# philipjesic/Distributed-Proof-Of-Work

Hardware: AMD Instinct MI355X
Metric: MD5 candidates/sec (GH/s), whole node (higher is better)
Workload: dtype u32; 1 GPU; sweep: nonce [1,2,3,4], 32 trailing zeros (unreachable), 2^36 candidates per GPU per step in the L=4 chunk segment (k >= 2^24); per-step RCCL MIN all-reduce; ntz=32, parallelism=prefix-partition x1 (workerBits=0)

## Files before the change

### distributed-proof-of-work_amd/csrc/md5_launch_ctl.h

```cpp
#pragma once
#include "md5_kernel_tune.h"

namespace dpow {
namespace DPOW_KNS {

constexpr uint32_t kTraceWaves = 8192;
constexpr uint32_t kTraceFields = 8;
#if DPOW_WAVE_TRACE
static __device__ unsigned long long g_wave_trace[kTraceWaves * kTraceFields];
#define DPOW_TRACED(...) { __VA_ARGS__ }
#else
#define DPOW_TRACED(...) {}
#endif
struct WaveTrace {
    unsigned long long t_start, t_first, n_wb, t_last, c_last, reason, t_hit, t_claims, t_bar;
    static DPOW_DEV unsigned long long now() { return __builtin_amdgcn_s_memrealtime(); }
    DPOW_DEV void start() DPOW_TRACED(t_start = now(); t_first = n_wb = t_last = c_last = reason = t_hit = 0;)
    DPOW_DEV void first_claim(uint64_t claim) DPOW_TRACED(t_first = now() + (claim & 0);)
    DPOW_DEV void chunk(uint64_t claim) DPOW_TRACED(t_last = now(); c_last = claim;)
    DPOW_DEV void wave_block() DPOW_TRACED(++n_wb;)
    DPOW_DEV void hit(bool h) DPOW_TRACED(if (h && t_hit == 0) t_hit = now();)
    DPOW_DEV void left(uint32_t why) DPOW_TRACED(reason = why;)
    DPOW_DEV void store(uint32_t lane) DPOW_TRACED(
        const uint32_t wave = (blockIdx.x - 1u) * (kBlockThreads / 64) + threadIdx.x / 64u;
        if (lane == 0 && wave < kTraceWaves) {
            unsigned long long *w = g_wave_trace + kTraceFields * wave;
            w[0] = t_start; w[1] = t_first; w[2] = now(); w[3] = n_wb;
            w[4] = t_last; w[5] = c_last; w[6] = reason; w[7] = t_hit;
        })
    DPOW_DEV void claims_performed() DPOW_TRACED(t_claims = now();)
    DPOW_DEV void barrier_passed() DPOW_TRACED(t_bar = now();)
    DPOW_DEV void counted(const Launch &L, uint32_t prev, uint32_t n) DPOW_TRACED(
        if (prev + n == L.done_target) {
            unsigned long long *r = g_wave_trace + kTraceFields * (kTraceWaves - 2);
            r[0] = t_claims; r[1] = t_bar; r[2] = now() + (prev & 0);
        })
    static DPOW_DEV void released() DPOW_TRACED(g_wave_trace[kTraceFields * (kTraceWaves - 2) + 3] = now();)
    static DPOW_DEV void watch(int f) DPOW_TRACED(
        unsigned long long *w = g_wave_trace + kTraceFields * (kTraceWaves - 1);
        if (f == 0 || f == 3 || w[f] == 0) w[f] = now();
        if (f == 0) w[1] = w[2] = 0;)
};
#undef DPOW_TRACED

__device__ __attribute__((noinline)) void publish(Ctrl *ctrl, Snap *snap, uint32_t seq, unsigned long long *claim,
                                                  Ctrl *ctrl_next) {
    if (ctrl_next == nullptr) {
        constexpr uintptr_t kRingBytes = kCtrlRing * kCtrlStride * sizeof(Ctrl);
        const uintptr_t a = reinterpret_cast<uintptr_t>(ctrl);
        ctrl_next =
            reinterpret_cast<Ctrl *>((a & ~(kRingBytes - 1)) | ((a + kCtrlStride * sizeof(Ctrl)) & (kRingBytes - 1)));
    }
    const unsigned long long t_start = __hip_atomic_load(&claim[1], __ATOMIC_RELAXED, __HIP_MEMORY_SCOPE_AGENT);
    for (uint32_t x = 0; x < kClaimCounters; ++x) claim[x * kClaimStride] = 0ull;
    claim[1] = 0ull;
    ctrl_next->best = kNoHit;
    ctrl_next->stop = 0u;
    ctrl_next->done = 0u;
    const unsigned long long best = __hip_atomic_load(&ctrl->best, __ATOMIC_RELAXED, __HIP_MEMORY_SCOPE_AGENT);
    const uint32_t stop = __hip_atomic_load(&ctrl->stop, __ATOMIC_RELAXED, __HIP_MEMORY_SCOPE_AGENT);
    __hip_atomic_store(&snap->best, best, __ATOMIC_RELAXED, __HIP_MEMORY_SCOPE_SYSTEM);
    __hip_atomic_store(&snap->stop, stop, __ATOMIC_RELAXED, __HIP_MEMORY_SCOPE_SYSTEM);
    __hip_atomic_store(&snap->t_start, t_start, __ATOMIC_RELAXED, __HIP_MEMORY_SCOPE_SYSTEM);
    __hip_atomic_store(&snap->t_end, __builtin_amdgcn_s_memrealtime(), __ATOMIC_RELAXED, __HIP_MEMORY_SCOPE_SYSTEM);
    __hip_atomic_store(&snap->seq, seq, __ATOMIC_RELEASE, __HIP_MEMORY_SCOPE_SYSTEM);
    WaveTrace::released();
}

DPOW_DEV void retire(const Launch &L, uint32_t done, Ctrl *ctrl_next) {
    if (done == L.done_target) publish(L.ctrl, L.snap, L.seq, L.claim, ctrl_next);
}

DPOW_DEV void watcher(const Launch &L) {
    if (threadIdx.x != 0) return;
    __hip_atomic_store(&L.claim[1], __builtin_amdgcn_s_memrealtime(), __ATOMIC_RELAXED, __HIP_MEMORY_SCOPE_AGENT);
    unsigned long long node_seen = ~0ull, bound_seen = L.bound0, early_seen = kNoHit;
    WaveTrace::watch(0);
    for (;;) {
        const unsigned long long *const nbp = L.node_best ? L.node_best : L.ext_bound;
        const uint32_t *const nsp = L.node_stop ? L.node_stop : L.cancel;
        const uint32_t done = __hip_atomic_load(&L.ctrl->done, __ATOMIC_RELAXED, __HIP_MEMORY_SCOPE_AGENT);
        const unsigned long long b = __hip_atomic_load(&L.ctrl->best, __ATOMIC_RELAXED, __HIP_MEMORY_SCOPE_AGENT);
        const uint32_t stale = __hip_atomic_load(L.stale, __ATOMIC_RELAXED, __HIP_MEMORY_SCOPE_SYSTEM);
        const uint32_t cancel = __hip_atomic_load(L.cancel, __ATOMIC_RELAXED, __HIP_MEMORY_SCOPE_SYSTEM);
        const unsigned long long eb = __hip_atomic_load(L.ext_bound, __ATOMIC_RELAXED, __HIP_MEMORY_SCOPE_SYSTEM);
        const unsigned long long nb = __hip_atomic_load(nbp, __ATOMIC_RELAXED, __HIP_MEMORY_SCOPE_SYSTEM);
        const uint32_t nstop = __hip_atomic_load(nsp, __ATOMIC_RELAXED, __HIP_MEMORY_SCOPE_SYSTEM);
        if (done >= L.done_target) {
            WaveTrace::watch(3);
            return;
        }
        if (L.early && b < early_seen) {
            WaveTrace::watch(2);
            early_seen = b;
            __hip_atomic_store(L.early, b, __ATOMIC_RELAXED, __HIP_MEMORY_SCOPE_SYSTEM);
        }
        bool stop = cancel != 0u || (int32_t)(stale - L.seq) >= 0;
        if (eb < bound_seen) {
            bound_seen = eb;
            __hip_atomic_fetch_min(&L.ctrl->best, eb, __ATOMIC_RELAXED, __HIP_MEMORY_SCOPE_AGENT);
        }
        if (L.node_best) {
            if (nb < node_seen) {
                if (nb < kNoHit) WaveTrace::watch(1);
                node_seen = nb;
                __hip_atomic_fetch_min(&L.ctrl->best, nb, __ATOMIC_RELAXED, __HIP_MEMORY_SCOPE_AGENT);
            }
            stop = stop || nstop != 0u;
        }
        if (stop) {
            __hip_atomic_store(&L.ctrl->stop, 1u, __ATOMIC_RELAXED, __HIP_MEMORY_SCOPE_AGENT);
            return;
        }
        __builtin_amdgcn_s_sleep(kWatchSleep);
    }
}

template <bool kOpaque>
DPOW_DEV unsigned long long claim_issue(unsigned long long *ctr, uint32_t lane) {
    unsigned long long v = 0;
    if constexpr (kOpaque) {
        uint32_t z;
        asm volatile("v_mov_b32 %0, 0" : "=v"(z));
        ctr += z;
    }
    if (lane == 0) v = __hip_atomic_fetch_add(ctr, 1ull, __ATOMIC_RELAXED, __HIP_MEMORY_SCOPE_AGENT);
    return v;
}

DPOW_DEV uint64_t claim_take(unsigned long long v, uint32_t x, uint64_t base) {
    const uint32_t lo = __builtin_amdgcn_readfirstlane((uint32_t)v);
    const uint32_t hi = __builtin_amdgcn_readfirstlane((uint32_t)(v >> 32));
    return (((uint64_t)hi << 32) | lo) * kClaimCounters + x + base;
}

DPOW_DEV uint64_t claim_next(unsigned long long *ctr, uint32_t x, uint32_t lane, uint64_t base) {
    return claim_take(claim_issue<false>(ctr, lane), x, base);
}

DPOW_DEV uint64_t lane_range_mask(int64_t lo, int64_t hi) {
    lo = lo < 0 ? 0 : (lo > 64 ? 64 : lo);
    hi = hi < 0 ? 0 : (hi > 64 ? 64 : hi);
    if (hi <= lo) return 0;
    const uint64_t upto_hi = hi == 64 ? ~0ull : ((1ull << hi) - 1ull);
    const uint64_t below_lo = lo == 64 ? ~0ull : ((1ull << lo) - 1ull);
    return upto_hi & ~below_lo;
}

}
}
```

### distributed-proof-of-work_amd/csrc/md5_search_si.h

```cpp
#pragma once

namespace dpow {
namespace DPOW_KNS {

constexpr uint32_t kSegLimitNone = 0xFFFFFFFFu;

DPOW_DEV uint64_t local_ceil_of_global(uint64_t g, uint32_t rbits, uint32_t base_tb) {
    const uint64_t k = g >> 8;
    const uint32_t tb = (uint32_t)(g & 0xFFu);
    if (tb < base_tb) return k << rbits;
    const uint32_t t = tb - base_tb;
    return t >> rbits ? (k + 1u) << rbits : (k << rbits) + t;
}

struct SegLimit {
    uint32_t q, r;
};
DPOW_DEV SegLimit seg_limit_of(const Launch &L, unsigned long long best) {
    const uint32_t segbits = 24u + L.rbits;
    const uint64_t ib = local_ceil_of_global(best, L.rbits, L.base_tb);
    const uint64_t rel = ib > L.wb_begin ? ib - L.wb_begin : 0ull;
    const uint64_t q = rel >> segbits;
    SegLimit l;
    l.q = q >= (uint64_t)kSegLimitNone ? kSegLimitNone - 1u : (uint32_t)q;
    l.r = (uint32_t)(rel - (q << segbits));
    return l;
}
DPOW_DEV uint32_t seg_limit_at(const SegLimit &l, uint32_t o) { return l.q + (o < l.r ? 1u : 0u); }

template <int NBLK, int W0, int SH>
DPOW_DEV void seg_invariants(uint32_t (&x)[4][kNC], uint32_t (&p)[kNC], const Launch &L, VarWords<true> &v) {
#pragma unroll
    for (int j = 0; j < kNC; ++j) {
        x[0][j] = L.iv[0]; x[1][j] = L.iv[1]; x[2][j] = L.iv[2]; x[3][j] = L.iv[3];
    }
    md5_steps<NBLK, W0, SH, 0, 0, W0 + 1, kNC>(x, L, v);
    using R = Roles<W0 + 1>;
#pragma unroll
    for (int j = 0; j < kNC; ++j) {
        p[j] = x[R::a][j] + md5_fn<W0 + 1>(x[R::b][j], x[R::c][j], x[R::d][j]);
        asm volatile("" : "+v"(p[j]), "+v"(x[Roles<W0>::a][j]));
        asm volatile("" : "+v"(v.w0km[1][j]), "+v"(v.w0km[2][j]), "+v"(v.w0km[3][j]));
    }
}

template <int NBLK, int W0, int SH>
DPOW_DEV uint64_t hash_wave_block_si(const Launch &L, const KConst &kc, const uint32_t (&xin)[4][kNC],
                                     const uint32_t (&p)[kNC], const VarWords<true> &v, const uint32_t (&vs)[kNC],
                                     uint32_t s, uint32_t o, uint32_t lane, uint32_t loff) {
    using K = VgprK<NBLK, W0, SH, true>;
    static_assert(K::Tune::kLead >= 2, "steps W0 and W0 + 1 precede the hand-ordered pipeline");
    uint32_t x[4][kNC];
#pragma unroll
    for (int j = 0; j < kNC; ++j)
#pragma unroll
        for (int w = 0; w < 4; ++w) x[w][j] = xin[w][j];
    {
        using R = Roles<W0 + 1>;
        const uint32_t km = L.KT[W0 + 1] + v.seg_d[0];
#pragma unroll
        for (int j = 0; j < kNC; ++j) x[R::a][j] = x[R::b][j] + __builtin_rotateleft32(p[j] + km, md5_shift(W0 + 1));
    }
    md5_steps<NBLK, W0, SH, 0, W0 + 2, K::kI0, kNC>(x, L, v);
    pipe::steps<NBLK, W0, SH, 0, K::kI0, K::kEnd0>(x, L, v);

    uint64_t bal[kNC];
    uint64_t any = 0;
#pragma unroll
    for (int j = 0; j < kNC; ++j) {
        bal[j] = __ballot(x[3][j] == L.deq);
        any |= bal[j];
    }
    if (any != 0) {
        const uint64_t i0 = L.wb_begin + ((uint64_t)s << (24u + L.rbits)) + o;
#pragma unroll
        for (int j = 0; j < kNC; ++j) {
            const uint64_t ij = i0 + 64u * j;
            uint64_t m = bal[j] & lane_range_mask((int64_t)(L.i_begin - ij), (int64_t)(L.i_end - ij));
            if (m != 0 && L.ntz > 8u) {
                const uint32_t sd[3] = {v.seg_d[0], 0u, 0u};
                const bool ok = ((m >> lane) & 1ull) && full_check<NBLK, W0, SH, true>(L, kc, vs[j], loff, sd);
                m = __ballot(ok);
            }
            if (m != 0) {
                const uint64_t g = global_of_local(ij + (uint64_t)__builtin_ctzll(m), L.rbits, L.base_tb);
                if (lane == 0) {
                    const unsigned long long prev = __hip_atomic_fetch_min(
                        &L.ctrl->best, (unsigned long long)g, __ATOMIC_RELAXED, __HIP_MEMORY_SCOPE_AGENT);
                    asm volatile("; dpow: atomicMin performed (%0)" ::"v"(prev));
                }
                return g;
            }
        }
    }
    return kNoHitG;
}

template <int NBLK, int W0, int SH, bool EQ>
DPOW_DEV void search_body_si(const Launch &L) {
    static_assert(NBLK == 1 && SH == 0 && EQ && W0 + 1 != 16 * NBLK - 2,
                  "segment-inner: one final block, SH = 0, D-equality, W0 + 1 not the bit-length word");
    if (blockIdx.x == 0) {
        watcher(L);
        return;
    }
    if constexpr (DPOW_SI_PAD > 0) asm volatile(".rept %0\n s_nop 0\n .endr" ::"i"(DPOW_SI_PAD));
    const uint32_t lane = threadIdx.x & 63u;
    const uint32_t loff = lane_offset(L.rbits, lane);
    KConst kc;
    kconst_init<NBLK, W0, SH, 0, 0, true>(kc, L);

    unsigned long long best = __hip_atomic_load(&L.ctrl->best, __ATOMIC_RELAXED, __HIP_MEMORY_SCOPE_AGENT);
    best = best < L.bound0 ? best : L.bound0;
    uint32_t stop = __hip_atomic_load(&L.ctrl->stop, __ATOMIC_RELAXED, __HIP_MEMORY_SCOPE_AGENT);

    __builtin_amdgcn_s_setprio(1);
    uint32_t x = (blockIdx.x - 1u) % kClaimCounters;
    const bool skip = stop != 0u || global_of_local(L.i_begin, L.rbits, L.base_tb) >= best;
    uint64_t claim = skip ? L.n_chunks : claim_next(L.claim + x * kClaimStride, x, lane, 0);
    const uint32_t segbits = 24u + L.rbits;
    SegLimit lim = seg_limit_of(L, best);
    uint32_t pc = L.poll_wb;
    unsigned long long best_seen = __hip_atomic_load(&L.ctrl->best, __ATOMIC_RELAXED, __HIP_MEMORY_SCOPE_AGENT);
    uint32_t stop_seen = __hip_atomic_load(&L.ctrl->stop, __ATOMIC_RELAXED, __HIP_MEMORY_SCOPE_AGENT);
    uint32_t hops = 0;
    for (;;) {
        if (claim >= L.n_chunks) {
            if (skip || ++hops >= kClaimCounters) break;
            x = (x + 1u) % kClaimCounters;
            const unsigned long long seen =
                __hip_atomic_load(L.claim + x * kClaimStride, __ATOMIC_RELAXED, __HIP_MEMORY_SCOPE_AGENT);
            claim = seen * kClaimCounters + x < L.n_chunks ? claim_next(L.claim + x * kClaimStride, x, lane, 0)
                                                           : L.n_chunks;
            continue;
        }
        unsigned long long next_v = 0;
        bool issued = false;
        const bool big = claim < L.n_big;
        if (!big) __builtin_amdgcn_s_setprio(0);
        const uint64_t b_begin = big ? claim * L.chunk : L.n_big * L.chunk + (claim - L.n_big) * L.chunk_tail;
        const uint32_t csz = big ? L.chunk : L.chunk_tail;
        const uint32_t nb = (uint32_t)(b_begin + csz < L.n_wblocks ? csz : L.n_wblocks - b_begin);
        uint32_t o = (uint32_t)(b_begin * (uint64_t)kWaveBlock);
        bool over = false;
        for (uint32_t left = nb; left != 0 && stop == 0u; --left, o += (uint32_t)kWaveBlock) {
            uint32_t s = L.wb_begin + o + (uint64_t)kWaveBlock <= L.i_begin ? 1u : 0u;
            const uint32_t s_hi =
                L.n_seg - (L.wb_begin + ((uint64_t)(L.n_seg - 1u) << segbits) + o >= L.i_end ? 1u : 0u);
            uint32_t s_end = seg_limit_at(lim, o);
            if (s_end == 0u) {
                over = true;
                break;
            }
            s_end = s_end < s_hi ? s_end : s_hi;
            if (left == 1u) {
                next_v = claim_issue<true>(L.claim + x * kClaimStride, lane);
                issued = true;
            }
            if (s >= s_end) continue;
            uint32_t vs[kNC];
            VarWords<true> v;
            v.kc = &kc;
            v.seg_d[0] = v.seg_d[1] = v.seg_d[2] = 0u;
#pragma unroll
            for (int j = 0; j < kNC; ++j) {
                vs[j] = wave_uniform_v(L.wb_begin + o + 64u * j, L.rbits, L.base_tb);
                var_words<SH>(v, j, vs[j], loff, 0u);
                w0km_fill<W0>(v, j, L);
            }
            uint32_t xin[4][kNC], p[kNC];
            seg_invariants<NBLK, W0, SH>(xin, p, L, v);
            for (; s < s_end; ++s) {
                v.seg_d[0] = s;
                if constexpr (DPOW_SI_VSEG != 0) {
                    const uint32_t d[3] = {s, 0u, 0u};
                    kconst_seg<NBLK, W0, SH, 0, 0, true>(kc, L, d);
                }
                const uint64_t g = hash_wave_block_si<NBLK, W0, SH>(L, kc, xin, p, v, vs, s, o, lane, loff);
                if (g != kNoHitG) {
                    best = g < best ? g : best;
                    lim = seg_limit_of(L, best);
                    s_end = s;
                }
                if (--pc == 0u) {
                    pc = L.poll_wb;
                    const bool lower = best_seen < best;
                    best = lower ? best_seen : best;
                    stop = stop_seen;
                    best_seen = __hip_atomic_load(&L.ctrl->best, __ATOMIC_RELAXED, __HIP_MEMORY_SCOPE_AGENT);
                    stop_seen = __hip_atomic_load(&L.ctrl->stop, __ATOMIC_RELAXED, __HIP_MEMORY_SCOPE_AGENT);
                    if (lower) {
                        lim = seg_limit_of(L, best);
                        const uint32_t e = seg_limit_at(lim, o);
                        s_end = e < s_end ? e : s_end;
                    }
                    if (stop != 0u) s_end = s;
                }
            }
        }
        if (stop != 0u || over || !issued) break;
        claim = claim_take(next_v, x, 0);
    }
    asm volatile("s_waitcnt vmcnt(0)" ::: "memory");
    __builtin_amdgcn_fence(__ATOMIC_RELEASE, "workgroup");
    __syncthreads();
    if (threadIdx.x == 0)
        retire(L, __hip_atomic_fetch_add(&L.ctrl->done, 1u, __ATOMIC_RELAXED, __HIP_MEMORY_SCOPE_AGENT) + 1u, L.ctrl_next);
}

}
}
```

### distributed-proof-of-work_amd/csrc/md5_variant.hip

```cpp
#include "md5_search_kernel.h"
#include "md5_variants.h"

#include <hip/hip_ext.h>

#ifndef DPOW_VNBLK
#error "DPOW_VNBLK must be defined"
#endif
#ifndef DPOW_VSH
#error "DPOW_VSH must be defined"
#endif

namespace dpow {

namespace {
using namespace DPOW_KNS;
using KernelFn = void (*)(Launch);
template <int NBLK, int W0, int SH, bool EQ, bool KSPAN>
constexpr KernelFn kernel_of() {
    constexpr int kSgpr = KernelTune<NBLK, W0, SH, KSPAN>::kSgpr;
    if constexpr (kSgpr == 2) return md5_search_kernel_w15sgpr<NBLK, W0, SH, EQ, KSPAN>;
    else if constexpr (kSgpr == 1) return md5_search_kernel_lsgpr<NBLK, W0, SH, EQ, KSPAN>;
    else return md5_search_kernel<NBLK, W0, SH, EQ, KSPAN>;
}
#define DPOW_K(w, e, nar) \
    kernel_of<DPOW_VNBLK, w, DPOW_VSH, e, !(DPOW_VSH == 3 && nar && narrow_knobs(DPOW_VNBLK, w).on)>()
#if DPOW_VSI
#if DPOW_VNBLK != 1 || DPOW_VSH != 0
#error "the segment-inner unit is built for NBLK = 1, SH = 0"
#endif
constexpr int kW0Lo = 0;
const KernelFn kTable[1][1][4] = {
    {{DPOW_K(0, true, false), DPOW_K(1, true, false), DPOW_K(2, true, false), DPOW_K(3, true, false)}}};
#define DPOW_ROW(e, n)
#elif DPOW_VNBLK == 1
constexpr int kW0Lo = 0;
#define DPOW_ROW(e, n)                                                                                              \
    {DPOW_K(0, e, n), DPOW_K(1, e, n), DPOW_K(2, e, n),  DPOW_K(3, e, n),  DPOW_K(4, e, n),  DPOW_K(5, e, n),        \
     DPOW_K(6, e, n), DPOW_K(7, e, n), DPOW_K(8, e, n),  DPOW_K(9, e, n),  DPOW_K(10, e, n), DPOW_K(11, e, n),       \
     DPOW_K(12, e, n), DPOW_K(13, e, n)}
const KernelFn kTable[2][2][14] = {{DPOW_ROW(false, false), DPOW_ROW(false, true)},
                                   {DPOW_ROW(true, false), DPOW_ROW(true, true)}};
#else
constexpr int kW0Lo = 12;
#define DPOW_ROW(e, n) {DPOW_K(12, e, n), DPOW_K(13, e, n), DPOW_K(14, e, n), DPOW_K(15, e, n)}
const KernelFn kTable[2][2][4] = {{DPOW_ROW(false, false), DPOW_ROW(false, true)},
                                  {DPOW_ROW(false, false), DPOW_ROW(false, true)}};
#endif
#undef DPOW_ROW
#undef DPOW_K
constexpr int kW0N = sizeof(kTable[0][0]) / sizeof(kTable[0][0][0]);

KernelFn pick(int w0, bool eq, bool narrow) {
#if DPOW_VSI
    return eq && w0 >= kW0Lo && w0 < kW0Lo + kW0N ? kTable[0][0][w0 - kW0Lo] : nullptr;
#endif
    return (w0 >= kW0Lo && w0 < kW0Lo + kW0N) ? kTable[eq ? 1 : 0][narrow ? 1 : 0][w0 - kW0Lo] : nullptr;
}
}

#if DPOW_VLS
#define DPOW_SFX _ls
#elif DPOW_VSI
#define DPOW_SFX _si
#else
#define DPOW_SFX
#endif
#define DPOW_CAT4(a, b, c, d) a##b##_##c##d
#define DPOW_NAME2(a, b, c, d) DPOW_CAT4(a, b, c, d)
#define DPOW_NAME(a, b, c) DPOW_NAME2(a, b, c, DPOW_SFX)

hipError_t DPOW_NAME(variant_launch_, DPOW_VNBLK, DPOW_VSH)(int w0, const Launch &L, uint32_t grid,
                                                           hipStream_t stream) {
    KernelFn fn = pick(w0, use_d_equality(DPOW_VNBLK, L.ntz), L.rbits >= 6u);
    if (!fn) return hipErrorInvalidValue;
    hipLaunchKernelGGL(fn, dim3(grid), dim3(kBlockThreads), 0, stream, L);
    return hipGetLastError();
}

hipError_t DPOW_NAME(variant_prepare_, DPOW_VNBLK, DPOW_VSH)() {
    for (const auto &eq : kTable)
        for (const auto &row : eq)
            for (KernelFn fn : row) {
                hipFuncAttributes a;
                const hipError_t e = hipFuncGetAttributes(&a, reinterpret_cast<const void *>(fn));
                if (e != hipSuccess) return e;
            }
    return hipSuccess;
}

hipError_t DPOW_NAME(variant_occupancy_, DPOW_VNBLK, DPOW_VSH)(int w0, int *blocks_per_cu) {
    KernelFn fn = pick(w0, DPOW_VSI != 0, true);
    if (!fn) return hipErrorInvalidValue;
    return hipOccupancyMaxActiveBlocksPerMultiprocessor(blocks_per_cu, reinterpret_cast<const void *>(fn),
                                                        kBlockThreads, 0);
}

}

#if DPOW_WAVE_TRACE && DPOW_VNBLK == 1 && DPOW_VSH == 0
#if DPOW_VLS
extern "C" int dpow_diag_wave_trace_ls(unsigned long long *out, size_t n) {
#else
extern "C" int dpow_diag_wave_trace(unsigned long long *out, size_t n) {
#endif
    if (n > dpow::DPOW_KNS::kTraceWaves * dpow::DPOW_KNS::kTraceFields)
        n = dpow::DPOW_KNS::kTraceWaves * dpow::DPOW_KNS::kTraceFields;
    return hipMemcpyFromSymbol(out, HIP_SYMBOL(dpow::DPOW_KNS::g_wave_trace), n * 8, 0, hipMemcpyDeviceToHost) == hipSuccess
               ? 0
               : -2;
}
#endif
```

### distributed-proof-of-work_amd/csrc/search.cpp

```cpp
#include <string.h>
#include <time.h>

#include <algorithm>

#include "ctx.h"
#include "md5_variants.h"

namespace dpow {

std::atomic<int> g_active[kMaxDevices];
std::mutex g_ctx_mu;
std::vector<dpow_ctx *> g_ctxs;

namespace {

constexpr int DPOW_BOUNDED = 3;

constexpr int64_t kSpinNs = 200000;
constexpr int64_t kSpinMaxNs = 4000000;
constexpr long kPollNs = 5000;
constexpr int64_t kNoDeadline = INT64_MAX;
constexpr int64_t kQueueLeadNs = 60000;
constexpr int64_t kEstFixedNs = 8000;

struct ActiveSearch {
    int dev;
    explicit ActiveSearch(int d) : dev(d) { g_active[dev].fetch_add(1, std::memory_order_relaxed); }
    ~ActiveSearch() { g_active[dev].fetch_sub(1, std::memory_order_relaxed); }
};

struct SearchWait {
    int64_t t0 = now_ns();
    int64_t spin_ns = kSpinNs;
    TimerSlack slack;
    uint64_t node_seen = DPOW_NO_HIT;
    bool node_stop = false;
    const uint64_t *early = nullptr;
    uint64_t early_seen = DPOW_NO_HIT;
    uint64_t own_posted = DPOW_NO_HIT;
    uint64_t covered = 0;
    const uint8_t *nonce = nullptr;
    size_t nonce_len = 0;
    uint32_t ntz = 0;
    uint32_t rbits = 8, base_tb = 0;
};

int poll_node(dpow_ctx *c, SearchWait &sw) {
    dpow_node_slot *n = c->node;
    if (!n) return 0;
    const uint64_t nb = __atomic_load_n(&n->best, __ATOMIC_ACQUIRE);
    if (nb < sw.node_seen) {
        sw.node_seen = nb;
        if (nb != sw.own_posted) {
            std::lock_guard<std::mutex> g(c->bound_mu);
            uint64_t cur = c->ext_bound.load(std::memory_order_relaxed);
            if (nb < cur) c->ext_bound.store(nb, std::memory_order_release);
        }
    }
    if (!sw.node_stop && __atomic_load_n(&n->stop, __ATOMIC_ACQUIRE) != 0u) {
        sw.node_stop = true;
        __atomic_store_n(&c->h_cancel[kStaleWord], (uint32_t)c->seq, __ATOMIC_RELEASE);
    }
    return 0;
}

void poll_early(dpow_ctx *c, SearchWait &sw) {
    const uint64_t g = __atomic_load_n(sw.early, __ATOMIC_ACQUIRE);
    if (g >= sw.early_seen) return;
    sw.early_seen = g;
    if ((((uint32_t)g & 0xFFu) >> sw.rbits) != (sw.base_tb >> sw.rbits)) return;
    uint8_t sec[DPOW_MAX_SECRET];
    size_t len = 0;
    if (dpow_secret_from_index(g, sec, &len) != 0) return;
    if (!dpow_verify(sw.nonce, sw.nonce_len, sec, len, sw.ntz)) return;
    if (g < sw.own_posted) sw.own_posted = g;
    dpow_node_post(c->node, g);
    if (c->diag_t[7] < 0) c->diag_t[7] = now_ns() - sw.t0;
}

int wait_record(dpow_ctx *c, uint64_t seq, int64_t deadline, SearchWait &sw) {
    const uint32_t *p = &c->h_snap[seq % kRing].seq;
    const uint32_t want = (uint32_t)(seq + 1);
    for (uint64_t it = 1;; ++it) {
        if (__atomic_load_n(p, __ATOMIC_ACQUIRE) == want) return 1;
        const int64_t t = now_ns();
        if (t >= deadline) return 0;
        const bool spinning = t - sw.t0 < sw.spin_ns;
        if (spinning ? (it % 4096 == 0) : (it % 16 == 0)) {
            const int alive = stream_liveness(c->slots[seq % kRing].stream, p, want,
                                              "dpow_search: stream idle without the launch's completion record");
            if (alive != 0) return alive;
        }
        if (sw.early && (!spinning || it % 8 == 0)) poll_early(c, sw);
        if (!spinning || it % 64 == 0) {
            if (c->node) {
                const int rc = poll_node(c, sw);
                if (rc < 0) return rc;
            }
            if (c->ext_bound.load(std::memory_order_acquire) <= sw.covered) return 2;
        }
        if (spinning) {
            __builtin_ia32_pause();
        } else {
            sw.slack.lower();
            int64_t ns = kPollNs;
            if (deadline != kNoDeadline && deadline - t < ns) ns = deadline - t;
            const struct timespec ts = {0, (long)ns};
            nanosleep(&ts, nullptr);
        }
    }
}

int retire_slot(dpow_ctx *c, LaunchSlot &s) {
    if (!s.in_flight) return 0;
    const uint32_t *p = &c->h_snap[s.seq % kRing].seq;
    const uint32_t want = (uint32_t)(s.seq + 1);
    for (uint64_t it = 1; __atomic_load_n(p, __ATOMIC_ACQUIRE) != want; ++it) {
        if (it % 1024 == 0) {
            const int alive = stream_liveness(s.stream, p, want,
                                              "dpow_search: stream idle without a queued launch's completion record");
            if (alive < 0) return alive;
            if (alive > 0) break;
        }
        __builtin_ia32_pause();
    }
    s.in_flight = false;
    return 0;
}

int recent_contexts(int device) {
    const int64_t t = now_ns();
    int n = 0;
    std::lock_guard<std::mutex> g(g_ctx_mu);
    for (dpow_ctx *x : g_ctxs)
        if (x->device == device && t - x->last_use.load(std::memory_order_relaxed) < kRecentNs) ++n;
    return n;
}

struct Search {
    dpow_ctx *const c;
    WindowPlanner &planner;
    const uint32_t ntz;
    const uint64_t bound;
    SearchWait sw;
    const uint64_t seq0 = c->seq;
    PlannedLaunch pl;
    bool have = false;
    size_t launched = 0, consumed = 0;
    int64_t busy_until = 0;
    Ctrl *const ctrl = c->d_ctrl + (size_t)c->ctrl_idx * kCtrlStride;
    Ctrl *const ctrl_next = c->d_ctrl + (size_t)((c->ctrl_idx + 1) % kCtrlRing) * kCtrlStride;
    bool md5_queued = false;
    uint64_t bound0 = DPOW_NO_HIT;
    bool window_open = false;
    uint32_t done_target = 0;
    uint64_t best = bound;

    Search(dpow_ctx *cc, WindowPlanner &p, uint32_t n, uint64_t b) : c(cc), planner(p), ntz(n), bound(b) {}
    ~Search() {
        if (consumed < launched) __atomic_store_n(&c->h_cancel[kStaleWord], (uint32_t)c->seq, __ATOMIC_RELEASE);
        if (window_open) {
            std::lock_guard<std::mutex> g(c->bound_mu);
            c->searching = false;
        }
        if (md5_queued) c->ctrl_idx = (c->ctrl_idx + 1) % kCtrlRing;
    }

    void queued(int32_t kind, uint64_t cands, uint64_t g_end) {
        const size_t li = launched++;
        const uint64_t seq = seq0 + li;
        if (li < dpow_ctx::kDiagLaunches) {
            c->diag_l[li] = {seq, cands, g_end, kind, now_ns(), -1};
            c->diag_nl = li + 1;
        }
        c->slots[seq % kRing] = {seq, true, cands, g_end, c->stream};
        c->seq = seq + 1;
    }

    void open_bound_window(uint64_t node_best) {
        bound0 = node_best < bound ? node_best : bound;
        std::lock_guard<std::mutex> g(c->bound_mu);
        c->ext_bound.store(node_best, std::memory_order_relaxed);
        __atomic_store_n(bound_word(c), (uint64_t)DPOW_NO_HIT, __ATOMIC_RELEASE);
        c->searching = true;
        window_open = true;
    }

    int queue_k0() {
        const int rc = retire_slot(c, c->slots[seq0 % kRing]);
        if (rc < 0) return rc;
        c->diag_t[5] = now_ns() - sw.t0;
        StartK0 k0{};
        k0.r = (uint32_t)(pl.L.i_end - pl.L.i_begin);
        k0.base_tb = pl.L.base_tb;
        k0.nblk = pl.info.nblk;
        k0.p = 4 * pl.info.w0 + pl.info.sh;
        k0.ntz = ntz;
        k0.seq = (uint32_t)(seq0 + 1);
        k0.snap = c->d_snap + seq0 % kRing;
        memcpy(k0.iv, pl.L.iv, sizeof k0.iv);
        memcpy(k0.T, pl.L.T, sizeof k0.T);
        const hipError_t e = search_k0(k0, c->stream);
        if (e != hipSuccess) return hip_fail(e, "search_k0");
        c->diag_t[0] = now_ns() - sw.t0;
        queued(0, k0.r, 1ull << 8);
        have = planner.next(pl);
        return 0;
    }

    int queue_md5() {
        const size_t li = launched;
        const uint64_t seq = seq0 + li;
        int rc = retire_slot(c, c->slots[seq % kRing]);
        if (rc < 0) return rc;
        if (!md5_queued) c->diag_t[6] = now_ns() - sw.t0;
        Launch &L = pl.L;
        uint64_t active = (uint64_t)std::max(1, g_active[c->device].load(std::memory_order_relaxed));
        if (active == 1 && !c->solo && now_ns() - sw.t0 < kYoungNs) {
            const int recent = recent_contexts(c->device);
            if (recent > 1) active = (uint64_t)recent;
        }
        uint64_t worker_blocks = 0;
        bool seg_inner = false;
        rc = size_window_launch(planner, pl, ntz, c->cus, active, c->knobs, &worker_blocks, &seg_inner);
        if (rc < 0) return set_error(rc, "dpow_search: launch grid leaves a claim counter without waves");
        done_target += (uint32_t)worker_blocks;
        L.claim = c->d_claims + (li % kClaimRing) * kClaimSlot;
        L.done_target = done_target;
        L.ctrl = ctrl;
        L.ctrl_next = ctrl_next;
        L.bound0 = bound0;
        L.cancel = c->d_cancel;
        L.stale = c->d_cancel + kStaleWord;
        L.ext_bound = reinterpret_cast<const unsigned long long *>(c->d_cancel + kBoundWord);
        L.snap = c->d_snap + seq % kRing;
        L.seq = (uint32_t)(seq + 1);
        L.node_best = c->d_node ? reinterpret_cast<const unsigned long long *>(&c->d_node->best) : nullptr;
        L.node_stop = c->d_node ? &c->d_node->stop : nullptr;
        L.early = c->d_node ? reinterpret_cast<unsigned long long *>(c->d_cancel + kEarlyWord) + c->ctrl_idx : nullptr;
        const hipError_t e = search_launch((int)pl.info.nblk, (int)pl.info.w0, (int)pl.info.sh, L,
                                           (uint32_t)(worker_blocks + 1), c->stream);
        if (e != hipSuccess) return hip_fail(e, "search_launch");
        if (!md5_queued) c->diag_t[1] = now_ns() - sw.t0;
        queued(L.n_seg != 0u ? 2 : 1, L.i_end - L.i_begin, pl.info.k_end << 8);
        md5_queued = true;
        const int64_t t = now_ns();
        busy_until = std::max(busy_until, t) + kEstFixedNs +
                     (int64_t)((double)(L.i_end - L.i_begin) * (double)active / kEstRate * 1e9);
        have = planner.next(pl);
        return 0;
    }

    int consume() {
        const size_t lj = consumed;
        const uint64_t seq = seq0 + lj;
        const int rc = wait_record(c, seq, kNoDeadline, sw);
        if (rc < 0) return rc;
        if (rc == 2) return DPOW_BOUNDED;
        LaunchSlot &slot = c->slots[seq % kRing];
        const Snap &sn = c->h_snap[seq % kRing];
        slot.in_flight = false;
        c->stats.launches++;
        c->stats.candidates += slot.candidates;
        if (sn.t_start != 0ull && sn.t_end >= sn.t_start)
            c->stats.kernel_ms += (double)(sn.t_end - sn.t_start) * kRealtimeNs * 1e-6;
        if (consumed == 0) c->diag_t[2] = now_ns() - sw.t0;
        if (lj < dpow_ctx::kDiagLaunches) c->diag_l[lj].seen = now_ns();
        consumed = lj + 1;
        if (c->node) {
            const int prc = poll_node(c, sw);
            if (prc < 0) return prc;
        }
        if (sn.best < bound) {
            const uint64_t eb = c->ext_bound.load(std::memory_order_acquire);
            if (sn.best >= eb) return eb <= slot.g_end ? DPOW_BOUNDED : DPOW_EXHAUSTED;
            best = sn.best;
            return DPOW_FOUND;
        }
        if (sn.stop != 0u || sw.node_stop || __atomic_load_n(c->h_cancel, __ATOMIC_ACQUIRE) != 0u)
            return DPOW_CANCELLED;
        sw.covered = slot.g_end;
        if (c->ext_bound.load(std::memory_order_acquire) <= sw.covered) return DPOW_BOUNDED;
        return DPOW_EXHAUSTED;
    }
};

}

int search_window(dpow_ctx *c, const uint8_t *nonce, size_t nonce_len, uint32_t ntz, uint32_t worker_byte,
                  uint32_t worker_bits, uint64_t k_begin, uint64_t k_end, uint64_t *best_global_idx,
                  uint8_t secret_out[DPOW_MAX_SECRET], size_t *secret_len) {
    WindowPlanner planner;
    int rc = planner.init(nonce, nonce_len, ntz, worker_byte, worker_bits, k_begin, k_end);
    if (rc < 0) return set_error(rc, "dpow_search: planning failed");
    const DeviceScope on_device(c->device);
    if (on_device.e != hipSuccess) return hip_fail(on_device.e, "hipSetDevice");
    if (c->device >= kMaxDevices) return set_error(DPOW_EINVAL, "dpow_search: device ordinal too large");
    const ActiveSearch active(c->device);
    Search s(c, planner, ntz, *best_global_idx);
    SearchWait &sw = s.sw;
    {
        const double searches = (double)std::max(1, g_active[c->device].load(std::memory_order_relaxed));
        const double expect_ns =
            (double)expected_first_hit(ntz, remainder_bits(worker_bits)) / kEstRate * 1e9 * searches;
        sw.spin_ns = expect_ns > 2.0 * (double)kSpinMaxNs
                         ? kSpinNs
                         : (int64_t)std::min<double>(std::max<double>(2.0 * expect_ns, (double)kSpinNs),
                                                     (double)kSpinMaxNs);
    }

    {
        uint32_t *st = &c->h_cancel[kStaleWord];
        const uint32_t next = (uint32_t)(c->seq + 1);
        if ((int32_t)(next - __atomic_load_n(st, __ATOMIC_RELAXED)) > (1 << 30))
            __atomic_store_n(st, next - (1u << 30), __ATOMIC_RELAXED);
    }
    const uint64_t node_best = c->node ? __atomic_load_n(&c->node->best, __ATOMIC_ACQUIRE) : DPOW_NO_HIT;
    sw.node_seen = node_best;
    sw.covered = k_begin << 8;
    for (int64_t &t : c->diag_t) t = -1;
    c->diag_nl = 0;
    c->diag_t0 = sw.t0;
    if (c->node) {
        uint64_t *ew = reinterpret_cast<uint64_t *>(c->h_cancel + kEarlyWord) + c->ctrl_idx;
        __atomic_store_n(ew, (uint64_t)DPOW_NO_HIT, __ATOMIC_RELEASE);
        sw.early = ew;
        sw.nonce = nonce;
        sw.nonce_len = nonce_len;
        sw.ntz = ntz;
        sw.rbits = remainder_bits(worker_bits);
        sw.base_tb = base_thread_byte(worker_byte, worker_bits);
    }
    s.have = planner.next(s.pl);
    c->diag_t[4] = now_ns() - sw.t0;
    if (s.have && s.pl.k0 && (rc = s.queue_k0()) < 0) return rc;
    s.open_bound_window(node_best);

    int status = DPOW_EXHAUSTED;
    while (status == DPOW_EXHAUSTED && s.have) {
        if (sw.node_stop) {
            status = DPOW_CANCELLED;
            break;
        }
        int w = 0;
        if (s.launched - s.consumed >= kDepth) {
            w = 1;
        } else if (s.launched > s.consumed && s.busy_until - now_ns() > kQueueLeadNs) {
            w = wait_record(c, s.seq0 + s.consumed, s.busy_until - kQueueLeadNs, sw);
            if (w < 0) return w;
        }
        if (w != 0) {
            const int r = w == 2 ? DPOW_BOUNDED : s.consume();
            if (r < 0) return r;
            if (r != DPOW_EXHAUSTED) status = r;
            continue;
        }
        {
            const uint64_t eb = c->ext_bound.load(std::memory_order_acquire);
            if ((s.pl.info.k_begin << 8) >= (eb < s.bound ? eb : s.bound)) break;
        }
        if ((rc = s.queue_md5()) < 0) return rc;
    }
    while (status == DPOW_EXHAUSTED && s.consumed < s.launched) {
        const int r = s.consume();
        if (r < 0) return r;
        status = r;
    }
    if (status == DPOW_BOUNDED) status = DPOW_EXHAUSTED;
    c->diag_t[3] = now_ns() - sw.t0;

    if (status == DPOW_FOUND) {
        dpow_secret_from_index(s.best, secret_out, secret_len);
        if (!dpow_verify(nonce, nonce_len, secret_out, *secret_len, ntz)) {
            *secret_len = 0;
            return set_error(DPOW_EVERIFY, "dpow_search: kernel hit failed host MD5 verification");
        }
        *best_global_idx = s.best;
    }
    return status;
}

}
```

Baseline: 229.8 GH/s.

## Prefetch stop/best poll loads, raise watcher priority, spin host after stop

After: 229.3 GH/s. Within noise of the previous version (-0.3%).

```diff
diff --git a/distributed-proof-of-work_amd/csrc/md5_launch_ctl.h b/distributed-proof-of-work_amd/csrc/md5_launch_ctl.h
--- a/distributed-proof-of-work_amd/csrc/md5_launch_ctl.h
+++ b/distributed-proof-of-work_amd/csrc/md5_launch_ctl.h
@@ -110,6 +110,7 @@
         }
         if (stop) {
             __hip_atomic_store(&L.ctrl->stop, 1u, __ATOMIC_RELAXED, __HIP_MEMORY_SCOPE_AGENT);
+            WaveTrace::watch(3);
             return;
         }
         __builtin_amdgcn_s_sleep(kWatchSleep);
diff --git a/distributed-proof-of-work_amd/csrc/md5_search_si.h b/distributed-proof-of-work_amd/csrc/md5_search_si.h
--- a/distributed-proof-of-work_amd/csrc/md5_search_si.h
+++ b/distributed-proof-of-work_amd/csrc/md5_search_si.h
@@ -28,6 +28,23 @@
 }
 DPOW_DEV uint32_t seg_limit_at(const SegLimit &l, uint32_t o) { return l.q + (o < l.r ? 1u : 0u); }
 
+struct PollLoads {
+    uint32_t lo, hi, stop;
+    DPOW_DEV void issue(const Ctrl *c) {
+        const unsigned long long b = __hip_atomic_load(&c->best, __ATOMIC_RELAXED, __HIP_MEMORY_SCOPE_AGENT);
+        lo = (uint32_t)b;
+        hi = (uint32_t)(b >> 32);
+        stop = __hip_atomic_load(&c->stop, __ATOMIC_RELAXED, __HIP_MEMORY_SCOPE_AGENT);
+    }
+    DPOW_DEV void take(unsigned long long &best_seen, uint32_t &stop_seen) {
+        asm volatile("" : "+v"(lo), "+v"(hi), "+v"(stop));
+        const uint32_t l = (uint32_t)__builtin_amdgcn_readfirstlane(lo);
+        const uint32_t h = (uint32_t)__builtin_amdgcn_readfirstlane(hi);
+        best_seen = ((unsigned long long)h << 32) | l;
+        stop_seen = (uint32_t)__builtin_amdgcn_readfirstlane(stop);
+    }
+};
+
 template <int NBLK, int W0, int SH>
 DPOW_DEV void seg_invariants(uint32_t (&x)[4][kNC], uint32_t (&p)[kNC], const Launch &L, VarWords<true> &v) {
 #pragma unroll
@@ -101,14 +118,18 @@
     static_assert(NBLK == 1 && SH == 0 && EQ && W0 + 1 != 16 * NBLK - 2,
                   "segment-inner: one final block, SH = 0, D-equality, W0 + 1 not the bit-length word");
     if (blockIdx.x == 0) {
+        __builtin_amdgcn_s_setprio(3);
         watcher(L);
         return;
     }
-    if constexpr (DPOW_SI_PAD > 0) asm volatile(".rept %0\n s_nop 0\n .endr" ::"i"(DPOW_SI_PAD));
+    constexpr int kPad = DPOW_SI_PAD > 0 ? DPOW_SI_PAD : W0 == 0 ? 1 : W0 == 1 ? 2 : W0 == 2 ? 3 : 6;
+    asm volatile(".rept %0\n s_nop 0\n .endr" ::"i"(kPad));
     const uint32_t lane = threadIdx.x & 63u;
     const uint32_t loff = lane_offset(L.rbits, lane);
     KConst kc;
     kconst_init<NBLK, W0, SH, 0, 0, true>(kc, L);
+    WaveTrace wt;
+    wt.start();
 
     unsigned long long best = __hip_atomic_load(&L.ctrl->best, __ATOMIC_RELAXED, __HIP_MEMORY_SCOPE_AGENT);
     best = best < L.bound0 ? best : L.bound0;
@@ -121,8 +142,8 @@
     const uint32_t segbits = 24u + L.rbits;
     SegLimit lim = seg_limit_of(L, best);
     uint32_t pc = L.poll_wb;
-    unsigned long long best_seen = __hip_atomic_load(&L.ctrl->best, __ATOMIC_RELAXED, __HIP_MEMORY_SCOPE_AGENT);
-    uint32_t stop_seen = __hip_atomic_load(&L.ctrl->stop, __ATOMIC_RELAXED, __HIP_MEMORY_SCOPE_AGENT);
+    PollLoads poll;
+    poll.issue(L.ctrl);
     uint32_t hops = 0;
     for (;;) {
         if (claim >= L.n_chunks) {
@@ -176,6 +197,7 @@
                     const uint32_t d[3] = {s, 0u, 0u};
                     kconst_seg<NBLK, W0, SH, 0, 0, true>(kc, L, d);
                 }
+                wt.wave_block();
                 const uint64_t g = hash_wave_block_si<NBLK, W0, SH>(L, kc, xin, p, v, vs, s, o, lane, loff);
                 if (g != kNoHitG) {
                     best = g < best ? g : best;
@@ -184,11 +206,12 @@
                 }
                 if (--pc == 0u) {
                     pc = L.poll_wb;
-                    const bool lower = best_seen < best;
+                    unsigned long long best_seen;
+                    uint32_t stop_seen;
+                    poll.take(best_seen, stop_seen);
+                    const bool lower = (long long)(best_seen - best) < 0;
                     best = lower ? best_seen : best;
                     stop = stop_seen;
-                    best_seen = __hip_atomic_load(&L.ctrl->best, __ATOMIC_RELAXED, __HIP_MEMORY_SCOPE_AGENT);
-                    stop_seen = __hip_atomic_load(&L.ctrl->stop, __ATOMIC_RELAXED, __HIP_MEMORY_SCOPE_AGENT);
                     if (lower) {
                         lim = seg_limit_of(L, best);
                         const uint32_t e = seg_limit_at(lim, o);
@@ -196,11 +219,14 @@
                     }
                     if (stop != 0u) s_end = s;
                 }
+                if (pc == 1u) poll.issue(L.ctrl);
             }
         }
         if (stop != 0u || over || !issued) break;
         claim = claim_take(next_v, x, 0);
     }
+    wt.left(stop != 0u ? 3 : 1);
+    wt.store(lane);
     asm volatile("s_waitcnt vmcnt(0)" ::: "memory");
     __builtin_amdgcn_fence(__ATOMIC_RELEASE, "workgroup");
     __syncthreads();
diff --git a/distributed-proof-of-work_amd/csrc/md5_variant.hip b/distributed-proof-of-work_amd/csrc/md5_variant.hip
--- a/distributed-proof-of-work_amd/csrc/md5_variant.hip
+++ b/distributed-proof-of-work_amd/csrc/md5_variant.hip
@@ -100,6 +100,8 @@
 #if DPOW_WAVE_TRACE && DPOW_VNBLK == 1 && DPOW_VSH == 0
 #if DPOW_VLS
 extern "C" int dpow_diag_wave_trace_ls(unsigned long long *out, size_t n) {
+#elif DPOW_VSI
+extern "C" int dpow_diag_wave_trace_si(unsigned long long *out, size_t n) {
 #else
 extern "C" int dpow_diag_wave_trace(unsigned long long *out, size_t n) {
 #endif
diff --git a/distributed-proof-of-work_amd/csrc/search.cpp b/distributed-proof-of-work_amd/csrc/search.cpp
--- a/distributed-proof-of-work_amd/csrc/search.cpp
+++ b/distributed-proof-of-work_amd/csrc/search.cpp
@@ -19,6 +19,7 @@
 constexpr int64_t kSpinNs = 200000;
 constexpr int64_t kSpinMaxNs = 4000000;
 constexpr long kPollNs = 5000;
+constexpr int64_t kStopSpinNs = 200000;
 constexpr int64_t kNoDeadline = INT64_MAX;
 constexpr int64_t kQueueLeadNs = 60000;
 constexpr int64_t kEstFixedNs = 8000;
@@ -35,6 +36,7 @@
     TimerSlack slack;
     uint64_t node_seen = DPOW_NO_HIT;
     bool node_stop = false;
+    int64_t stop_t = -1;
     const uint64_t *early = nullptr;
     uint64_t early_seen = DPOW_NO_HIT;
     uint64_t own_posted = DPOW_NO_HIT;
@@ -78,6 +80,11 @@
     if (c->diag_t[7] < 0) c->diag_t[7] = now_ns() - sw.t0;
 }
 
+bool stop_known(const dpow_ctx *c, uint32_t want, const SearchWait &sw) {
+    return sw.node_stop || __atomic_load_n(c->h_cancel, __ATOMIC_ACQUIRE) != 0u ||
+           (int32_t)(__atomic_load_n(&c->h_cancel[kStaleWord], __ATOMIC_ACQUIRE) - want) >= 0;
+}
+
 int wait_record(dpow_ctx *c, uint64_t seq, int64_t deadline, SearchWait &sw) {
     const uint32_t *p = &c->h_snap[seq % kRing].seq;
     const uint32_t want = (uint32_t)(seq + 1);
@@ -85,7 +92,8 @@
         if (__atomic_load_n(p, __ATOMIC_ACQUIRE) == want) return 1;
         const int64_t t = now_ns();
         if (t >= deadline) return 0;
-        const bool spinning = t - sw.t0 < sw.spin_ns;
+        if (sw.stop_t < 0 && stop_known(c, want, sw)) sw.stop_t = t;
+        const bool spinning = t - sw.t0 < sw.spin_ns || (sw.stop_t >= 0 && t - sw.stop_t < kStopSpinNs);
         if (spinning ? (it % 4096 == 0) : (it % 16 == 0)) {
             const int alive = stream_liveness(c->slots[seq % kRing].stream, p, want,
                                               "dpow_search: stream idle without the launch's completion record");
```
